# princeton-vl/DROID-SLAM

Measured on NVIDIA B200. Metric: BA-update iters/sec (512 edges, 344x64x48), higher is better.
Workload: dtype f32 (BA solve in f64), f16 corr volumes

## Files before the change

droid_slam_b200/csrc/ba.cu:

```cuda
#include "common.cuh"
#include "tcgen05.cuh"
#include <math.h>
#include <algorithm>

namespace dba {

constexpr int kBuildThreads = 256;
constexpr int kEdgeBatch = 16;

struct Layout {
  size_t off_hdr, off_frame2k, off_kx, off_rowptr, off_edgeidx, off_big, off_sys, off_L, off_dx, off_Eij, off_C, off_w, off_Ei, total;
  int P, n;
};

__host__ inline size_t align_up(size_t x, size_t a) { return (x + a - 1) / a * a; }

__host__ inline Layout make_layout(int N, int E, int ht, int wd, int t0, int t1) {
  Layout L;
  const size_t HW = (size_t)ht * wd;
  L.P = t1 - t0 > 0 ? t1 - t0 : 0;
  L.n = 6 * L.P;
  size_t o = 0;
  L.off_hdr = o;      o = align_up(o + 64 * sizeof(int), 256);
  L.off_frame2k = o;  o = align_up(o + (size_t)(N + 1) * sizeof(int), 256);
  L.off_kx = o;       o = align_up(o + (size_t)(N + 1) * sizeof(int), 256);
  L.off_rowptr = o;   o = align_up(o + (size_t)(N + 2) * sizeof(int), 256);
  L.off_edgeidx = o;  o = align_up(o + (size_t)(E + 1) * sizeof(int), 256);
  L.off_big = o;      o = align_up(o + (size_t)(N + 1) * sizeof(int), 256);
  L.off_sys = o;      o = align_up(o + ((size_t)L.n * L.n + L.n) * sizeof(double), 256);
  L.off_L = o;        o = align_up(o + chol_workspace_bytes(L.n), 256);
  L.off_dx = o;       o = align_up(o + (size_t)(L.n + 6) * sizeof(float), 256);
  L.off_Eij = o;      o = align_up(o + (size_t)E * 6 * HW * sizeof(float), 256);
  const size_t Mmax = (size_t)N;
  L.off_C = o;        o = align_up(o + Mmax * HW * sizeof(float), 256);
  L.off_w = o;        o = align_up(o + Mmax * HW * sizeof(float), 256);
  L.off_Ei = o;       o = align_up(o + Mmax * 6 * HW * sizeof(float), 256);
  L.total = o;
  return L;
}

enum { HDR_STATUS = 0, HDR_M = 1, HDR_CHOL_FAIL = 2, HDR_NBIG = 3 };
enum { ST_BAD_INDEX = 1, ST_ETA_ROWS = 2, ST_CHOL_FAIL = 4, ST_DEGREE = 8 };

__global__ void __launch_bounds__(1024) ba_prepare_kernel(const int64_t* __restrict__ ii, const int64_t* __restrict__ jj, int E, int N,
                                                          int t0, int t1, int eta_rows, int* __restrict__ hdr,
                                                          int* __restrict__ frame2k, int* __restrict__ kx, int* __restrict__ rowptr, int* __restrict__ big) {
  __shared__ int s_scan[1024];
  __shared__ int s_carry;
  const int tid = threadIdx.x;
  if (tid == 0) { hdr[HDR_STATUS] = 0; hdr[HDR_CHOL_FAIL] = 0; }
  for (int f = tid; f < N; f += blockDim.x) { frame2k[f] = (f >= t0 && f < t1) ? 1 : 0; rowptr[f] = 0; }
  if (tid == 0) { rowptr[N] = 0; rowptr[N + 1] = 0; }
  __syncthreads();
  for (int e = tid; e < E; e += blockDim.x) {
    const long long i = ii[e], j = jj[e];
    if (i < 0 || i >= N || j < 0 || j >= N) { atomicOr(&hdr[HDR_STATUS], ST_BAD_INDEX); continue; }
    frame2k[i] = 1;
  }
  __syncthreads();
  if (tid == 0) s_carry = 0;
  __syncthreads();
  for (int base = 0; base < N; base += blockDim.x) {
    const int f = base + tid;
    const int flag = (f < N) ? frame2k[f] : 0;
    s_scan[tid] = flag;
    __syncthreads();
    for (int off = 1; off < (int)blockDim.x; off <<= 1) {
      int v = (tid >= off) ? s_scan[tid - off] : 0;
      __syncthreads();
      s_scan[tid] += v;
      __syncthreads();
    }
    const int incl = s_scan[tid];
    const int idx = s_carry + incl - flag;
    if (f < N) {
      frame2k[f] = flag ? idx : -1;
      if (flag) kx[idx] = f;
    }
    __syncthreads();
    if (tid == blockDim.x - 1) s_carry += incl;
    __syncthreads();
  }
  const int M = s_carry;
  if (tid == 0) {
    hdr[HDR_M] = M;
    if (eta_rows != M && eta_rows != 1) atomicOr(&hdr[HDR_STATUS], ST_ETA_ROWS);
  }
  for (int e = tid; e < E; e += blockDim.x) {
    const long long i = ii[e], j = jj[e];
    if (i < 0 || i >= N || j < 0 || j >= N) continue;
    atomicAdd(&rowptr[frame2k[i] + 1], 1);
  }
  __syncthreads();
  if (tid == 0) s_carry = 0;
  __syncthreads();
  for (int base = 0; base <= M; base += blockDim.x) {
    const int m = base + tid;
    const int cnt = (m <= M) ? rowptr[m] : 0;
    s_scan[tid] = cnt;
    __syncthreads();
    for (int off = 1; off < (int)blockDim.x; off <<= 1) {
      int v = (tid >= off) ? s_scan[tid - off] : 0;
      __syncthreads();
      s_scan[tid] += v;
      __syncthreads();
    }
    if (m <= M) rowptr[m] = s_carry + s_scan[tid];
    __syncthreads();
    if (tid == blockDim.x - 1) s_carry += s_scan[tid];
    __syncthreads();
  }
  if (tid == 0) s_carry = 0;
  __syncthreads();
  for (int base = 0; base < M; base += blockDim.x) {
    const int m = base + tid;
    const int flag = (m < M && rowptr[m + 1] - rowptr[m] + 1 > 21) ? 1 : 0;
    s_scan[tid] = flag;
    __syncthreads();
    for (int off = 1; off < (int)blockDim.x; off <<= 1) {
      int v = (tid >= off) ? s_scan[tid - off] : 0;
      __syncthreads();
      s_scan[tid] += v;
      __syncthreads();
    }
    if (flag) big[s_carry + s_scan[tid] - 1] = m;
    __syncthreads();
    if (tid == blockDim.x - 1) s_carry += s_scan[tid];
    __syncthreads();
  }
  if (tid == 0) hdr[HDR_NBIG] = s_carry;
}

__global__ void __launch_bounds__(256) ba_fill_csr_kernel(const int64_t* __restrict__ ii, const int64_t* __restrict__ jj, int E, int N,
                                                          const int* __restrict__ frame2k, const int* __restrict__ rowptr,
                                                          int* __restrict__ edgeidx) {
  const int e = (blockIdx.x * blockDim.x + threadIdx.x) >> 5;
  const int lane = threadIdx.x & 31;
  if (e >= E) return;
  const long long i = ii[e], j = jj[e];
  if (i < 0 || i >= N || j < 0 || j >= N) return;
  int rank = 0;
  for (int f = lane; f < e; f += 32) {
    const long long i2 = ii[f], j2 = jj[f];
    rank += (i2 == i && j2 >= 0 && j2 < N) ? 1 : 0;
  }
// ... 22 lines not shown
  int e, jx, stereo;
};

__device__ __forceinline__ void adj_se3(const float* t, const float* q, const float* X, float* Y) {
  float qinv[4] = {-q[0], -q[1], -q[2], q[3]};
  act_so3(qinv, X, Y);
  act_so3(qinv, X + 3, Y + 3);
  float u[3], v[3];
  u[0] = t[2] * X[1] - t[1] * X[2];
  u[1] = t[0] * X[2] - t[2] * X[0];
  u[2] = t[1] * X[0] - t[0] * X[1];
  act_so3(qinv, u, v);
  Y[3] += v[0]; Y[4] += v[1]; Y[5] += v[2];
}

template <int kPPT>
__global__ void __launch_bounds__(kBuildThreads, 2) ba_build_kernel(
    const float* __restrict__ poses, const float* __restrict__ disps, const float* __restrict__ intr,
    const float* __restrict__ disps_sens, const float* __restrict__ targets, const float* __restrict__ weights,
    const float* __restrict__ eta, int eta_rows, int eta_by_frame, const int64_t* __restrict__ jj,
    const int* __restrict__ hdr, const int* __restrict__ kx, const int* __restrict__ rowptr, const int* __restrict__ edgeidx,
    int HW, int wd, int t0, int P, int motion_only,
    double* __restrict__ Hsys, double* __restrict__ bsys, float* __restrict__ Eij, float* __restrict__ Cout, float* __restrict__ wout,
    float* __restrict__ Eiout) {
  const int m = blockIdx.y;
  if (m >= hdr[HDR_M]) return;
  const int ix = kx[m];
  const int e_begin = rowptr[m], e_end = rowptr[m + 1];
  const int tid = threadIdx.x, lane = tid & 31, warp = tid >> 5;
  constexpr int NW = kBuildThreads / 32;

  __shared__ EdgeSm s_edge[kEdgeBatch];
  __shared__ float s_part[NW][kEdgeBatch][27];
  __shared__ double s_sum[kEdgeBatch][27];

  const float fx = __ldg(intr), fy = __ldg(intr + 1), cx = __ldg(intr + 2), cy = __ldg(intr + 3);
  const int n = 6 * P;

  int pix[kPPT];
  float Xi0[kPPT], Xi1[kPPT], dsp[kPPT];
  float Cacc[kPPT], wacc[kPPT], Eiacc[kPPT][6];
#pragma unroll
  for (int s = 0; s < kPPT; s++) {
    const int p = blockIdx.x * (kPPT * kBuildThreads) + s * kBuildThreads + tid;
    pix[s] = p;
    const bool ok = p < HW;
    const int i = ok ? p / wd : 0, j = ok ? p - i * wd : 0;
    Xi0[s] = ((float)j - cx) / fx;
    Xi1[s] = ((float)i - cy) / fy;
    dsp[s] = ok ? __ldg(disps + (size_t)ix * HW + p) : 1.f;
    Cacc[s] = 0.f; wacc[s] = 0.f;
#pragma unroll
    for (int c = 0; c < 6; c++) Eiacc[s][c] = 0.f;
  }

  for (int eb = e_begin; eb < e_end; eb += kEdgeBatch) {
    const int nb = min(kEdgeBatch, e_end - eb);
    __syncthreads();
    if (tid < nb) {
// ... 163 lines not shown
#pragma unroll
    for (int s = 0; s < kPPT; s++) {
      const int p = pix[s];
      if (p < HW) {
        const float dsn = __ldg(disps_sens + (size_t)ix * HW + p);
        const float mk = (dsn > 0.f) ? 1.f : 0.f;
        const float C = Cacc[s] + mk * alpha + (1 - mk) * __ldg(eta + (size_t)erow * HW + p);
        const float w = wacc[s] - mk * alpha * (dsp[s] - dsn);
        Cout[(size_t)m * HW + p] = C;
        wout[(size_t)m * HW + p] = w;
#pragma unroll
        for (int c = 0; c < 6; c++) Eiout[((size_t)m * 6 + c) * HW + p] = Eiacc[s][c];
      }
    }
  }
}

__device__ __forceinline__ float safe_rcp(float c) { return c > 0.f ? 1.0f / c : 0.f; }

constexpr int kSchurMaxRows = 255;

template <int kThreads>
__device__ __forceinline__ void build_row_list(const int64_t* __restrict__ jj, int* __restrict__ hdr, const int* __restrict__ edgeidx,
                                               int e_begin, int deg, int ix, int m, int HW, int t0, int P, const float* __restrict__ Eij,
                                               const float* __restrict__ Eiin, int* s_pose, const float** s_ptr, int* s_nrows, int* s_wcount) {
  const int tid = threadIdx.x, lane = tid & 31, warp = tid >> 5;
  const bool self = (ix >= t0 && ix < t0 + P);
  int pj = -1, e = -1;
  if (tid < deg && tid < kSchurMaxRows - 1) { e = edgeidx[e_begin + tid]; pj = (int)jj[e] - t0; }
  const bool keep = (pj >= 0 && pj < P);
  const unsigned bal = __ballot_sync(0xffffffffu, keep);
  if (lane == 0) s_wcount[warp] = __popc(bal);
  __syncthreads();
  int base = self ? 1 : 0;
  for (int w = 0; w < warp; w++) base += s_wcount[w];
// ... 280 lines not shown
    if (o < 36) {
      const int a = o / 6, c = o - a * 6;
      const int gr = pa_ * 6 + a, gc = pb_ * 6 + c;
      if (same_row) {
        if (gr >= gc) atomicAdd(&Hsys[(size_t)gr * n + gc], v);
      } else {
        if (gr >= gc) atomicAdd(&Hsys[(size_t)gr * n + gc], v);
        if (gc >= gr) atomicAdd(&Hsys[(size_t)gc * n + gr], v);
      }
    } else {
      atomicAdd(&bsys[pa_ * 6 + (o - 36)], v);
    }
  }
}

constexpr int kTcRowsMax = 21;
constexpr int kPairTileRows = 10;
constexpr int kPairRowsMax = 100;
constexpr int kPairGridZ = 45;
constexpr int kTcThreads = 288;
constexpr int kTcProducers = 256;
constexpr int kTcRawStages = 4;
constexpr int kTcRawBytes = 128 * 128;
constexpr int kTcOpBytes = 128 * 128;
constexpr int kTcOpStages = 4;
constexpr int kTcAccSlots = 3;
constexpr int kTcCxStride = 129;
constexpr int kTcSmem = kTcRawStages * kTcRawBytes + kTcOpStages * 2 * kTcOpBytes + 1024  + 256 ;
static_assert(128 * kTcCxStride * 4 <= kTcOpStages * 2 * kTcOpBytes, "G staging matrix must fit the operand ring");

__device__ __forceinline__ void cp_async16_zfill(uint32_t dst, const void* src, uint32_t src_bytes) {
  asm volatile("cp.async.cg.shared.global [%0], [%1], 16, %2;" ::"r"(dst), "l"(src), "r"(src_bytes) : "memory");
}
__device__ __forceinline__ float lds_f32(uint32_t addr) {
  float v;
  asm volatile("ld.shared.f32 %0, [%1];" : "=f"(v) : "r"(addr) : "memory");
  return v;
}
__device__ __forceinline__ void sts_f32(uint32_t addr, float v) { asm volatile("st.shared.f32 [%0], %1;" ::"r"(addr), "f"(v) : "memory"); }

template <bool PAIR>
__global__ void __launch_bounds__(kTcThreads, 1) ba_schur_tc_kernel(
    const int64_t* __restrict__ jj, int* __restrict__ hdr, const int* __restrict__ kx, const int* __restrict__ rowptr,
    const int* __restrict__ edgeidx, int HW, int t0, int P, int px_per_cta,
    const float* __restrict__ Eij, const float* __restrict__ Cin, const float* __restrict__ win, const float* __restrict__ Eiin,
    double* __restrict__ Hsys, double* __restrict__ bsys, const int* __restrict__ big) {
  if (PAIR && (int)blockIdx.y >= hdr[HDR_NBIG]) return;
  const int m = PAIR ? big[blockIdx.y] : blockIdx.y;
  if (m >= hdr[HDR_M]) return;
  const int ix = kx[m];
  const int e_begin = rowptr[m];
  const int deg = rowptr[m + 1] - e_begin;
  const int tid = threadIdx.x, lane = tid & 31, warp = tid >> 5;
  const int n = 6 * P;

  __shared__ int s_pose[kSchurMaxRows + 1];
  __shared__ const float* s_ptr[kSchurMaxRows + 1];
  __shared__ int s_nrows;
  __shared__ int s_wcount[kTcThreads / 32];
  __shared__ int s_gidx[128];
  extern __shared__ uint8_t tc_smem_raw[];

  if (deg == 0) return;
  if (PAIR) {
    if (deg + 1 <= kTcRowsMax) return;
    const int tmax = (min(deg + 1, kPairRowsMax) + kPairTileRows - 1) / kPairTileRows;
    if ((int)blockIdx.z >= tmax * (tmax - 1) / 2) return;
  }
  build_row_list<kTcThreads>(jj, hdr, edgeidx, e_begin, deg, ix, m, HW, t0, P, Eij, Eiin, s_pose, s_ptr, &s_nrows, s_wcount);
  const int nrows = s_nrows;
  if (!PAIR && (nrows == 0 || nrows > kTcRowsMax)) return;
  if (PAIR && (nrows <= kTcRowsMax || nrows > kPairRowsMax)) return;
  int ta = 0, tb = 0;
  bool emit_a = true, emit_b = true;
  if (PAIR) {
    const int T = (nrows + kPairTileRows - 1) / kPairTileRows;
    const int pr = blockIdx.z;
    if (pr >= T * (T - 1) / 2) return;
    tb = (int)((sqrtf(8.f * (float)pr + 1.f) + 1.f) * 0.5f);
    while (tb * (tb - 1) / 2 > pr) tb--;
    while ((tb + 1) * tb / 2 <= pr) tb++;
    ta = pr - tb * (tb - 1) / 2;
    emit_a = (tb == ta + 1);
    emit_b = (tb == T - 1 && ta == T - 2);
  }
  const int px_begin = blockIdx.x * px_per_cta;
  const int px_end = min(HW, px_begin + px_per_cta);
  if (px_begin >= px_end) return;
  const int R6a = PAIR ? 6 * min(kPairTileRows, nrows - kPairTileRows * ta) : 6 * nrows;
  const int R6b = PAIR ? 6 * min(kPairTileRows, nrows - kPairTileRows * tb) : 6 * nrows;
  const int R6 = R6a;
  const bool packed = !PAIR && (R6 + 2 <= 64);
  const bool two_halves = PAIR || packed;
  const int nhalf = packed ? 2 : 1;
  const int cpx = 32 * nhalf;
  const int nchunks = (px_end - px_begin + cpx - 1) / cpx;
  const int N = two_halves ? 128 : ((R6 + 1 + 15) & ~15);

  uint8_t* smem = reinterpret_cast<uint8_t*>((reinterpret_cast<uintptr_t>(tc_smem_raw) + 1023) & ~(uintptr_t)1023);
  const uint32_t op_base = smem_u32(smem);
  const uint32_t raw_base = op_base + kTcOpStages * 2 * kTcOpBytes;
  uint64_t* bars = reinterpret_cast<uint64_t*>(smem + kTcOpStages * 2 * kTcOpBytes + kTcRawStages * kTcRawBytes);
  uint64_t* full = bars;
  uint64_t* empty = bars + kTcOpStages;
  uint64_t* acc_full = bars + 2 * kTcOpStages;
  uint64_t* acc_empty = acc_full + kTcAccSlots;
  uint64_t* done = acc_empty + kTcAccSlots;
  uint32_t* tmem_base_smem = reinterpret_cast<uint32_t*>(done + 2);

  if (tid < 128) {
    if (PAIR) {
      const int hfx = tid >> 6, ln = tid & 63, R6x = hfx ? R6b : R6a, row0 = kPairTileRows * (hfx ? tb : ta);
      s_gidx[tid] = (ln < R6x) ? s_pose[row0 + ln / 6] * 6 + (ln % 6) : (ln == R6x ? -1 : -2);
    } else s_gidx[tid] = (tid < R6) ? s_pose[tid / 6] * 6 + (tid % 6) : (tid == R6 ? -1 : -2);
  }
  if (tid == 0) {
    for (int s = 0; s < kTcOpStages; s++) { mbar_init(full + s, kTcProducers / 32); mbar_init(empty + s, 1); }
    for (int s = 0; s < kTcAccSlots; s++) { mbar_init(acc_full + s, 1); mbar_init(acc_empty + s, kTcProducers / 32); }
    mbar_init(done, 1);
    asm volatile("fence.mbarrier_init.release.cluster;" ::: "memory");
  }
  if (warp == 8) {
    asm volatile("tcgen05.alloc.cta_group::1.sync.aligned.shared::cta.b32 [%0], 512;" ::"r"(smem_u32(tmem_base_smem)) : "memory");
    asm volatile("tcgen05.relinquish_alloc_permit.cta_group::1.sync.aligned;" ::: "memory");
  } else {
    uint4* z = reinterpret_cast<uint4*>(smem);
    for (int k = tid; k < kTcOpStages * 2 * kTcOpBytes / 16; k += kTcProducers) z[k] = make_uint4(0u, 0u, 0u, 0u);
  }
  asm volatile("tcgen05.fence::before_thread_sync;" ::: "memory");
  __syncthreads();
  asm volatile("tcgen05.fence::after_thread_sync;" ::: "memory");
  const uint32_t tmem_base = *tmem_base_smem;

  if (warp == 8) {
    if (lane == 0) {
      const uint32_t idesc = umma_idesc_tf32(128, N);
      const uint32_t d_g = tmem_base + 3 * 128;
      for (int c = 0; c < nchunks; c++) {
        const int os = c % kTcOpStages, slot = c % kTcAccSlots;
        mbar_wait(full + os, (c / kTcOpStages) & 1);
        if (c >= kTcAccSlots) mbar_wait(acc_empty + slot, ((c / kTcAccSlots) - 1) & 1);
        asm volatile("tcgen05.fence::after_thread_sync;" ::: "memory");
        const uint32_t hi0 = op_base + (uint32_t)os * 2 * kTcOpBytes, lo0 = hi0 + kTcOpBytes;
        const uint32_t d = tmem_base + (uint32_t)(slot * 128);
#pragma unroll
        for (int k = 0; k < 4; k++) {
          const uint64_t dh = umma_desc_k_sw128(hi0 + k * 32, 1024), dl = umma_desc_k_sw128(lo0 + k * 32, 1024);
          umma_tf32(d, dh, dh, idesc, k > 0 ? 1u : 0u);
          umma_tf32(d_g, dh, dl, idesc, (c > 0 || k > 0) ? 1u : 0u);
        }
        umma_commit(empty + os);
        umma_commit(acc_full + slot);
      }
      umma_commit(done);
    }
    __syncwarp();
  } else {
    const float* src[4];
    uint32_t dst[4];
    int pxo[4];
#pragma unroll
    for (int i = 0; i < 4; i++) {
      const int li = 4 * i + (lane >> 3), piece = lane & 7;
      const int hf = two_halves ? (li >> 3) : 0, line = warp + 8 * (two_halves ? (li & 7) : li);
      const int R6x = PAIR ? (hf ? R6b : R6a) : R6, row0 = PAIR ? kPairTileRows * (hf ? tb : ta) : 0;
      src[i] = Cin; pxo[i] = 1 << 30;
      dst[i] = raw_base + warp * 2048 + li * 128 + piece * 16;
      if (line <= R6x) {
        const float* base = (line < R6x) ? s_ptr[row0 + line / 6] + (size_t)(line % 6) * HW : win + (size_t)m * HW;
// ... 143 lines not shown
              if (gr > gc) atomicAdd(&Hsys[(size_t)gr * n + gc], v);
              else if (gr < gc) atomicAdd(&Hsys[(size_t)gc * n + gr], v);
              else atomicAdd(&Hsys[(size_t)gr * n + gr], 2.0 * v);
            } else if (gc >= 0) {
              if (gr >= gc) atomicAdd(&Hsys[(size_t)gr * n + gc], v);
            } else {
              atomicAdd(&bsys[gr], v);
            }
          }
        }
      }
    }
  }
  asm volatile("tcgen05.fence::before_thread_sync;" ::: "memory");
  __syncthreads();
  if (warp == 8) asm volatile("tcgen05.dealloc.cta_group::1.sync.aligned.b32 %0, 512;" ::"r"(tmem_base) : "memory");
}

__device__ __forceinline__ void exp_so3(const float* phi, float* q) {
  const float theta_sq = phi[0] * phi[0] + phi[1] * phi[1] + phi[2] * phi[2];
  const float theta_p4 = theta_sq * theta_sq;
  const float theta = sqrtf(theta_sq);
  float imag, real;
  if ((double)theta_sq < 1e-8) {
    imag = (float)(0.5 - (1.0 / 48.0) * (double)theta_sq + (1.0 / 3840.0) * (double)theta_p4);
    real = (float)(1.0 - (1.0 / 8.0) * (double)theta_sq + (1.0 / 384.0) * (double)theta_p4);
  } else {
    imag = (float)((double)sinf((float)(0.5 * (double)theta)) / (double)theta);
    real = cosf((float)(0.5 * (double)theta));
  }
// ... 107 lines not shown
  DBA_CHECK_ARG(a->p2p_world <= 8 && (a->p2p_world <= 1 || (a->p2p_rank >= 0 && a->p2p_rank < a->p2p_world)), "bad p2p rank/world");
  DBA_CHECK_ARG(a->workspace != nullptr, "null workspace");
  DBA_CHECK_ARG(a->n_frames <= 65535, "more than 65535 frames");
  L = make_layout(a->n_frames, a->n_edges, a->ht, a->wd, a->t0, a->t1);
  if (a->workspace_bytes < L.total) { dba::set_error("workspace too small: %zu < %zu", a->workspace_bytes, L.total); return DBA_ERR_WORKSPACE; }
  return DBA_OK;
}

#define WS(T, off) reinterpret_cast<T*>(reinterpret_cast<char*>(a->workspace) + (off))

static double* system_ptr(const dba_ba_args* a, const Layout& L) {
  if (a->p2p_world > 1) return reinterpret_cast<double*>(a->p2p_system[a->p2p_rank]) + (size_t)(a->p2p_epoch & 1ull) * ((size_t)L.n * L.n + L.n);
  return reinterpret_cast<double*>(reinterpret_cast<char*>(a->workspace) + L.off_sys);
}

extern "C" int dba_ba_prepare(const dba_ba_args* a) {
  Layout L; int rc = check_ba_args(a, L); if (rc) return rc;
  cudaStream_t st = (cudaStream_t)a->stream;
  ba_prepare_kernel<<<1, 1024, 0, st>>>(a->ii, a->jj, a->n_edges, a->n_frames, a->t0, a->t1, (a->motion_only || a->eta_by_frame) ? 1 : a->eta_rows,
                                        WS(int, L.off_hdr), WS(int, L.off_frame2k), WS(int, L.off_kx), WS(int, L.off_rowptr), WS(int, L.off_big));
  DBA_CHECK_LAUNCH("ba_prepare");
  if (a->n_edges > 0) {
    ba_fill_csr_kernel<<<(a->n_edges + 7) / 8, 256, 0, st>>>(a->ii, a->jj, a->n_edges, a->n_frames, WS(int, L.off_frame2k),
                                                                  WS(int, L.off_rowptr), WS(int, L.off_edgeidx));
    DBA_CHECK_LAUNCH("ba_fill_csr");
  }
  return DBA_OK;
}

extern "C" int dba_ba_build(const dba_ba_args* a) {
  Layout L; int rc = check_ba_args(a, L); if (rc) return rc;
  cudaStream_t st = (cudaStream_t)a->stream;
  const int HW = a->ht * a->wd;
  double* Hsys = system_ptr(a, L);
  double* bsys = Hsys + (size_t)L.n * L.n;
  DBA_CHECK_CUDA(cudaMemsetAsync(Hsys, 0, ((size_t)L.n * L.n + L.n) * sizeof(double), st), "ba_build memset");
  DBA_CHECK_CUDA(cudaMemsetAsync(WS(int, L.off_hdr) + HDR_CHOL_FAIL, 0, sizeof(int), st), "ba_build memset");
  if (L.P == 0) return DBA_OK;
  const int eff_frames = std::max(1, std::min(a->n_frames, a->own_hi - a->own_lo));
  const int ppt = (eff_frames * ((HW + 4 * kBuildThreads - 1) / (4 * kBuildThreads)) >= 148) ? 4
                : (eff_frames * ((HW + 2 * kBuildThreads - 1) / (2 * kBuildThreads)) >= 148) ? 2 : 1;
#define LAUNCH_BUILD(PPT)                                                                                                               \
  ba_build_kernel<PPT><<<dim3((HW + PPT * kBuildThreads - 1) / (PPT * kBuildThreads), a->n_frames), kBuildThreads, 0, st>>>(             \
      a->poses, a->disps, a->intrinsics, a->disps_sens, a->targets, a->weights, a->eta, a->eta_rows, a->eta_by_frame, a->jj, WS(int, L.off_hdr),  \
      WS(int, L.off_kx), WS(int, L.off_rowptr), WS(int, L.off_edgeidx), HW, a->wd, a->t0, L.P, a->motion_only, Hsys, bsys,               \
      WS(float, L.off_Eij), WS(float, L.off_C), WS(float, L.off_w), WS(float, L.off_Ei))
  if (ppt == 4) LAUNCH_BUILD(4); else if (ppt == 2) LAUNCH_BUILD(2); else LAUNCH_BUILD(1);
#undef LAUNCH_BUILD
  DBA_CHECK_LAUNCH("ba_build");
  if (!a->motion_only) {
    const size_t smem2 = (size_t)2 * kSgK * kSgStride * sizeof(float);
    const int tiles1 = (HW + kSgK - 1) / kSgK;
    const int chunks1 = std::max(1, std::min(tiles1, (5 * 148 / 2 + eff_frames - 1) / eff_frames));
    const int px_per_cta1 = ((tiles1 + chunks1 - 1) / chunks1) * kSgK;
    const int gx1 = (HW + px_per_cta1 - 1) / px_per_cta1;
    const int px_per_cta2 = ((HW + 2) / 3 + kSgK - 1) / kSgK * kSgK;
    const int gx2 = (HW + px_per_cta2 - 1) / px_per_cta2;
    const int zsplit2 = std::max(1, std::min(32, (6 * 148 + eff_frames * gx2 - 1) / (eff_frames * gx2)));
    if ((rc = kernel_setup((const void*)ba_schur_gemm_kernel, (int)smem2))) return rc;
    if ((rc = kernel_setup((const void*)ba_schur_small_kernel, (int)smem2))) return rc;
    if ((rc = kernel_setup((const void*)ba_schur_tc_kernel<false>, (int)kTcSmem))) return rc;
    if ((rc = kernel_setup((const void*)ba_schur_tc_kernel<true>, (int)kTcSmem))) return rc;
    const bool use_tc = HW % 4 == 0;
    if (use_tc) {
      const int tiles64 = (HW + 63) / 64;
      const int chunks_tc = std::max(1, std::min(tiles64, (148 + eff_frames / 2) / eff_frames));
      const int px_per_cta_tc = ((tiles64 + chunks_tc - 1) / chunks_tc) * 64;
      const int gx_tc = (HW + px_per_cta_tc - 1) / px_per_cta_tc;
      ba_schur_tc_kernel<false><<<dim3(gx_tc, a->n_frames, 1), kTcThreads, kTcSmem, st>>>(a->jj, WS(int, L.off_hdr), WS(int, L.off_kx), WS(int, L.off_rowptr),
                                                           WS(int, L.off_edgeidx), HW, a->t0, L.P, px_per_cta_tc, WS(float, L.off_Eij),
                                                           WS(float, L.off_C), WS(float, L.off_w), WS(float, L.off_Ei), Hsys, bsys, WS(int, L.off_big));
      const int max_big = std::min(a->n_frames, a->n_edges / kTcRowsMax);
      if (max_big > 0)
        ba_schur_tc_kernel<true><<<dim3(1, max_big, kPairGridZ), kTcThreads, kTcSmem, st>>>(a->jj, WS(int, L.off_hdr), WS(int, L.off_kx), WS(int, L.off_rowptr),
                                                           WS(int, L.off_edgeidx), HW, a->t0, L.P, ((HW + 31) / 32) * 32, WS(float, L.off_Eij),
                                                           WS(float, L.off_C), WS(float, L.off_w), WS(float, L.off_Ei), Hsys, bsys, WS(int, L.off_big));
    } else {
      ba_schur_small_kernel<<<dim3(gx1, a->n_frames, 1), kSgThreads, smem2, st>>>(a->jj, WS(int, L.off_hdr), WS(int, L.off_kx), WS(int, L.off_rowptr),
                                                           WS(int, L.off_edgeidx), HW, a->t0, L.P, px_per_cta1, WS(float, L.off_Eij),
                                                           WS(float, L.off_C), WS(float, L.off_w), WS(float, L.off_Ei), Hsys, bsys);
    }
    DBA_CHECK_LAUNCH("ba_schur<single>");
    ba_schur_gemm_kernel<<<dim3(gx2, a->n_frames, zsplit2), kSgThreads, smem2, st>>>(a->jj, WS(int, L.off_hdr), WS(int, L.off_kx), WS(int, L.off_rowptr),
                                                                         WS(int, L.off_edgeidx), HW, a->t0, L.P, px_per_cta2, use_tc ? kPairRowsMax : kSgRows, WS(float, L.off_Eij),
                                                                         WS(float, L.off_C), WS(float, L.off_w), WS(float, L.off_Ei), Hsys, bsys);
    DBA_CHECK_LAUNCH("ba_schur<multi>");
  }
  return DBA_OK;
}

extern "C" int dba_ba_solve(const dba_ba_args* a) {
// ... 78 lines not shown
```

Before: 873.1.

## Use persistent work-queue kernels for BA build and tensor-core Schur stages

```diff
diff --git a/droid_slam_b200/csrc/ba.cu b/droid_slam_b200/csrc/ba.cu
--- a/droid_slam_b200/csrc/ba.cu
+++ b/droid_slam_b200/csrc/ba.cu
@@ -2,16 +2,31 @@
 #include "tcgen05.cuh"
 #include <math.h>
 #include <algorithm>
+#include <climits>
 
 namespace dba {
 
 constexpr int kBuildThreads = 256;
 constexpr int kEdgeBatch = 16;
+constexpr int kPPT = 4;
+constexpr int kBuildCtasPerSm = 2;
+constexpr int kSchurMaxRows = 255;
+constexpr int kTcPackedRowsMax = 10;
+constexpr int kTcRowsMax = 21;
+constexpr int kPairTileRows = 10;
+constexpr int kPairRowsMax = 100;
+constexpr int kTcItemOverhead = 4;
 
 struct Layout {
-  size_t off_hdr, off_frame2k, off_kx, off_rowptr, off_edgeidx, off_big, off_sys, off_L, off_dx, off_Eij, off_C, off_w, off_Ei, total;
+  size_t off_hdr, off_frame2k, off_kx, off_rowptr, off_edgeidx, off_rows, off_work, off_bwork, off_sys, off_L, off_dx, off_Eij, off_C, off_w, off_Ei, total;
   int P, n;
 };
+
+constexpr int kTcRangesMax = 64;
+constexpr int kPairItemsMax = 45;
+__host__ inline size_t tc_work_capacity(int N, int E) {
+  return (size_t)N * kTcRangesMax + (size_t)std::min(N, E / 21) * kPairItemsMax;
+}
 
 __host__ inline size_t align_up(size_t x, size_t a) { return (x + a - 1) / a * a; }
 
@@ -26,7 +41,9 @@
   L.off_kx = o;       o = align_up(o + (size_t)(N + 1) * sizeof(int), 256);
   L.off_rowptr = o;   o = align_up(o + (size_t)(N + 2) * sizeof(int), 256);
   L.off_edgeidx = o;  o = align_up(o + (size_t)(E + 1) * sizeof(int), 256);
-  L.off_big = o;      o = align_up(o + (size_t)(N + 1) * sizeof(int), 256);
+  L.off_rows = o;     o = align_up(o + (size_t)(N + 1) * sizeof(int), 256);
+  L.off_work = o;     o = align_up(o + tc_work_capacity(N, E) * sizeof(int4), 256);
+  L.off_bwork = o;    o = align_up(o + (size_t)N * ((HW + 255) / 256) * sizeof(int4), 256);
   L.off_sys = o;      o = align_up(o + ((size_t)L.n * L.n + L.n) * sizeof(double), 256);
   L.off_L = o;        o = align_up(o + chol_workspace_bytes(L.n), 256);
   L.off_dx = o;       o = align_up(o + (size_t)(L.n + 6) * sizeof(float), 256);
@@ -39,96 +56,168 @@
   return L;
 }
 
-enum { HDR_STATUS = 0, HDR_M = 1, HDR_CHOL_FAIL = 2, HDR_NBIG = 3 };
+enum { HDR_STATUS = 0, HDR_M = 1, HDR_CHOL_FAIL = 2, HDR_NEXT = 3, HDR_BNEXT = 4, HDR_NWORK = 5, HDR_NBWORK = 6 };
 enum { ST_BAD_INDEX = 1, ST_ETA_ROWS = 2, ST_CHOL_FAIL = 4, ST_DEGREE = 8 };
 
+__device__ __forceinline__ int block_scan_excl(int v, int* s_warp, int* total) {
+  const int tid = threadIdx.x, lane = tid & 31, warp = tid >> 5;
+  int x = v;
+#pragma unroll
+  for (int o = 1; o < 32; o <<= 1) { const int y = __shfl_up_sync(0xffffffffu, x, o); if (lane >= o) x += y; }
+  if (lane == 31) s_warp[warp] = x;
+  __syncthreads();
+  if (warp == 0) {
+    int w = s_warp[lane];
+#pragma unroll
+    for (int o = 1; o < 32; o <<= 1) { const int y = __shfl_up_sync(0xffffffffu, w, o); if (lane >= o) w += y; }
+    s_warp[lane] = w - s_warp[lane];
+    if (lane == 31) s_warp[32] = w;
+  }
+  __syncthreads();
+  const int r = s_warp[warp] + x - v;
+  *total = s_warp[32];
+  __syncthreads();
+  return r;
+}
+
+__device__ __forceinline__ int tc_chunks(int R, int deg, int HW) {
+  if (deg == 0 || deg > kSchurMaxRows - 1 || R == 0 || R > kTcRowsMax) return 0;
+  return R <= kTcPackedRowsMax ? (HW + 63) / 64 : (HW + 31) / 32;
+}
+__device__ __forceinline__ int tc_pairs(int R, int deg) {
+  if (deg > kSchurMaxRows - 1 || R <= kTcRowsMax || R > kPairRowsMax) return 0;
+  const int T = (R + kPairTileRows - 1) / kPairTileRows;
+  return T * (T - 1) / 2;
+}
+
+__device__ __forceinline__ int build_ppt(int deg, int cmax4) {
+  return (deg * 4 <= cmax4) ? 4 : (deg * 2 <= cmax4) ? 2 : 1;
+}
+
 __global__ void __launch_bounds__(1024) ba_prepare_kernel(const int64_t* __restrict__ ii, const int64_t* __restrict__ jj, int E, int N,
-                                                          int t0, int t1, int eta_rows, int* __restrict__ hdr,
-                                                          int* __restrict__ frame2k, int* __restrict__ kx, int* __restrict__ rowptr, int* __restrict__ big) {
-  __shared__ int s_scan[1024];
-  __shared__ int s_carry;
+                                                          int t0, int t1, int eta_rows, int HW, int tc_grid, int build_slots,
+                                                          int* __restrict__ hdr, int* __restrict__ frame2k, int* __restrict__ kx,
+                                                          int* __restrict__ rowptr, int* __restrict__ rows, int4* __restrict__ work,
+                                                          int4* __restrict__ bwork) {
+  __shared__ int s_warp[33];
+  __shared__ int s_cnt[2];
+  __shared__ int s_cpi;
   const int tid = threadIdx.x;
-  if (tid == 0) { hdr[HDR_STATUS] = 0; hdr[HDR_CHOL_FAIL] = 0; }
-  for (int f = tid; f < N; f += blockDim.x) { frame2k[f] = (f >= t0 && f < t1) ? 1 : 0; rowptr[f] = 0; }
+  const int nthr = blockDim.x;
+  if (tid == 0) { hdr[HDR_STATUS] = 0; hdr[HDR_CHOL_FAIL] = 0; s_cnt[0] = 0; s_cnt[1] = 0; }
+  for (int f = tid; f < N; f += nthr) { frame2k[f] = (f >= t0 && f < t1) ? 1 : 0; rowptr[f] = 0; }
   if (tid == 0) { rowptr[N] = 0; rowptr[N + 1] = 0; }
   __syncthreads();
-  for (int e = tid; e < E; e += blockDim.x) {
+  for (int e = tid; e < E; e += nthr) {
     const long long i = ii[e], j = jj[e];
     if (i < 0 || i >= N || j < 0 || j >= N) { atomicOr(&hdr[HDR_STATUS], ST_BAD_INDEX); continue; }
     frame2k[i] = 1;
   }
   __syncthreads();
-  if (tid == 0) s_carry = 0;
-  __syncthreads();
-  for (int base = 0; base < N; base += blockDim.x) {
+  int carry = 0, tot;
+  for (int base = 0; base < N; base += nthr) {
     const int f = base + tid;
     const int flag = (f < N) ? frame2k[f] : 0;
-    s_scan[tid] = flag;
-    __syncthreads();
-    for (int off = 1; off < (int)blockDim.x; off <<= 1) {
-      int v = (tid >= off) ? s_scan[tid - off] : 0;
-      __syncthreads();
-      s_scan[tid] += v;
-      __syncthreads();
-    }
-    const int incl = s_scan[tid];
-    const int idx = s_carry + incl - flag;
+    const int idx = carry + block_scan_excl(flag, s_warp, &tot);
     if (f < N) {
       frame2k[f] = flag ? idx : -1;
       if (flag) kx[idx] = f;
     }
-    __syncthreads();
-    if (tid == blockDim.x - 1) s_carry += incl;
-    __syncthreads();
-  }
-  const int M = s_carry;
+    carry += tot;
+  }
+  const int M = carry;
   if (tid == 0) {
     hdr[HDR_M] = M;
     if (eta_rows != M && eta_rows != 1) atomicOr(&hdr[HDR_STATUS], ST_ETA_ROWS);
   }
-  for (int e = tid; e < E; e += blockDim.x) {
+  __syncthreads();
+  for (int m = tid; m < M; m += nthr) rows[m] = (kx[m] >= t0 && kx[m] < t1) ? 1 : 0;
+  __syncthreads();
+  for (int e = tid; e < E; e += nthr) {
     const long long i = ii[e], j = jj[e];
     if (i < 0 || i >= N || j < 0 || j >= N) continue;
     atomicAdd(&rowptr[frame2k[i] + 1], 1);
-  }
-  __syncthreads();
-  if (tid == 0) s_carry = 0;
-  __syncthreads();
-  for (int base = 0; base <= M; base += blockDim.x) {
+    if (j >= t0 && j < t1) atomicAdd(&rows[frame2k[i]], 1);
+  }
+  __syncthreads();
+  carry = 0;
+  for (int base = 0; base <= M; base += nthr) {
     const int m = base + tid;
     const int cnt = (m <= M) ? rowptr[m] : 0;
-    s_scan[tid] = cnt;
-    __syncthreads();
-    for (int off = 1; off < (int)blockDim.x; off <<= 1) {
-      int v = (tid >= off) ? s_scan[tid - off] : 0;
-      __syncthreads();
-      s_scan[tid] += v;
-      __syncthreads();
-    }
-    if (m <= M) rowptr[m] = s_carry + s_scan[tid];
-    __syncthreads();
-    if (tid == blockDim.x - 1) s_carry += s_scan[tid];
-    __syncthreads();
-  }
-  if (tid == 0) s_carry = 0;
-  __syncthreads();
-  for (int base = 0; base < M; base += blockDim.x) {
-    const int m = base + tid;
-    const int flag = (m < M && rowptr[m + 1] - rowptr[m] + 1 > 21) ? 1 : 0;
-    s_scan[tid] = flag;
-    __syncthreads();
-    for (int off = 1; off < (int)blockDim.x; off <<= 1) {
-      int v = (tid >= off) ? s_scan[tid - off] : 0;
-      __syncthreads();
-      s_scan[tid] += v;
-      __syncthreads();
-    }
-    if (flag) big[s_carry + s_scan[tid] - 1] = m;
-    __syncthreads();
-    if (tid == blockDim.x - 1) s_carry += s_scan[tid];
-    __syncthreads();
-  }
-  if (tid == 0) hdr[HDR_NBIG] = s_carry;
+    const int incl = carry + block_scan_excl(cnt, s_warp, &tot) + cnt;
+    if (m <= M) rowptr[m] = incl;
+    carry += tot;
+  }
+  __syncthreads();
+
+  {
+    int w = 0;
+    for (int m = tid; m < M; m += nthr) w += max(1, rowptr[m + 1] - rowptr[m]);
+    const int chunks4 = (HW + 1023) / 1024;
+    int wsum = 0;
+    block_scan_excl(w, s_warp, &wsum);
+    const int cmax4 = max(16, (int)(4LL * wsum * chunks4 / max(1, build_slots)));
+    carry = 0;
+    for (int base = 0; base < M; base += nthr) {
+      const int m = base + tid;
+      int cnt = 0, px = 0;
+      if (m < M) {
+        px = 256 * build_ppt(rowptr[m + 1] - rowptr[m], cmax4);
+        cnt = (HW + px - 1) / px;
+      }
+      const int first = carry + block_scan_excl(cnt, s_warp, &tot);
+      for (int r = 0; r < cnt; r++) bwork[first + r] = make_int4(m, r * px, min(HW, (r + 1) * px), 0);
+      carry += tot;
+    }
+    if (tid == 0) hdr[HDR_NBWORK] = carry;
+  }
+
+  if (tc_grid <= 0) { if (tid == 0) hdr[HDR_NWORK] = 0; return; }
+  for (int m = tid; m < M; m += nthr) {
+    const int R = rows[m], deg = rowptr[m + 1] - rowptr[m];
+    if (tc_chunks(R, deg, HW)) atomicAdd(&s_cnt[R <= kTcPackedRowsMax ? 0 : 1], 1);
+  }
+  __syncthreads();
+  if (tid < 32) {
+    const int cp = (HW + 63) / 64, cu = (HW + 31) / 32;
+    const int cpi_min = (cu + kTcRangesMax - 1) / kTcRangesMax;
+    long long best_cost = LLONG_MAX; int best = 0;
+    for (int c = tid + 1; c <= 64; c += 32) {
+      const long long items = (long long)s_cnt[0] * ((cp + c - 1) / c) + (long long)s_cnt[1] * ((cu + c - 1) / c);
+      const long long cost = c < cpi_min ? LLONG_MAX : (items + tc_grid - 1) / tc_grid * (c + kTcItemOverhead);
+      if (cost < best_cost || (cost == best_cost && c > best)) { best_cost = cost; best = c; }
+    }
+#pragma unroll
+    for (int o = 16; o > 0; o >>= 1) {
+      const long long oc = __shfl_xor_sync(0xffffffffu, best_cost, o);
+      const int ob = __shfl_xor_sync(0xffffffffu, best, o);
+      if (oc < best_cost || (oc == best_cost && ob > best)) { best_cost = oc; best = ob; }
+    }
+    if (tid == 0) s_cpi = max(best, cpi_min);
+  }
+  __syncthreads();
+  const int cpi = s_cpi;
+  carry = 0;
+  for (int pass = 0; pass < 2; pass++) {
+    for (int base = 0; base < M; base += nthr) {
+      const int m = base + tid;
+      int cnt = 0, R = 0, deg = 0;
+      if (m < M) {
+        R = rows[m]; deg = rowptr[m + 1] - rowptr[m];
+        cnt = pass == 0 ? tc_pairs(R, deg) : (tc_chunks(R, deg, HW) + cpi - 1) / cpi;
+      }
+      const int first = carry + block_scan_excl(cnt, s_warp, &tot);
+      if (pass == 0) {
+        for (int z = 0; z < cnt; z++) work[first + z] = make_int4(m, 0, HW, z);
+      } else if (cnt > 0) {
+        const int c = tc_chunks(R, deg, HW), cpx = R <= kTcPackedRowsMax ? 64 : 32;
+        for (int r = 0; r < cnt; r++)
+          work[first + r] = make_int4(m, (int)((long long)r * c / cnt) * cpx, min(HW, (int)((long long)(r + 1) * c / cnt) * cpx), -1);
+      }
+      carry += tot;
+    }
+  }
+  if (tid == 0) hdr[HDR_NWORK] = carry;
 }
 
 __global__ void __launch_bounds__(256) ba_fill_csr_kernel(const int64_t* __restrict__ ii, const int64_t* __restrict__ jj, int E, int N,
@@ -181,35 +270,43 @@
   Y[3] += v[0]; Y[4] += v[1]; Y[5] += v[2];
 }
 
-template <int kPPT>
-__global__ void __launch_bounds__(kBuildThreads, 2) ba_build_kernel(
+__global__ void __launch_bounds__(kBuildThreads, kBuildCtasPerSm) ba_build_kernel(
     const float* __restrict__ poses, const float* __restrict__ disps, const float* __restrict__ intr,
     const float* __restrict__ disps_sens, const float* __restrict__ targets, const float* __restrict__ weights,
     const float* __restrict__ eta, int eta_rows, int eta_by_frame, const int64_t* __restrict__ jj,
-    const int* __restrict__ hdr, const int* __restrict__ kx, const int* __restrict__ rowptr, const int* __restrict__ edgeidx,
+    int* __restrict__ hdr, const int* __restrict__ kx, const int* __restrict__ rowptr, const int* __restrict__ edgeidx,
     int HW, int wd, int t0, int P, int motion_only,
     double* __restrict__ Hsys, double* __restrict__ bsys, float* __restrict__ Eij, float* __restrict__ Cout, float* __restrict__ wout,
-    float* __restrict__ Eiout) {
-  const int m = blockIdx.y;
-  if (m >= hdr[HDR_M]) return;
-  const int ix = kx[m];
-  const int e_begin = rowptr[m], e_end = rowptr[m + 1];
+    float* __restrict__ Eiout, const int4* __restrict__ bwork) {
   const int tid = threadIdx.x, lane = tid & 31, warp = tid >> 5;
   constexpr int NW = kBuildThreads / 32;
 
   __shared__ EdgeSm s_edge[kEdgeBatch];
   __shared__ float s_part[NW][kEdgeBatch][27];
   __shared__ double s_sum[kEdgeBatch][27];
+  __shared__ int s_item;
 
   const float fx = __ldg(intr), fy = __ldg(intr + 1), cx = __ldg(intr + 2), cy = __ldg(intr + 3);
   const int n = 6 * P;
+  const int nwork = hdr[HDR_NBWORK];
+  for (;;) {
+  __syncthreads();
+  if (tid == 0) s_item = atomicAdd(&hdr[HDR_BNEXT], 1);
+  __syncthreads();
+  const int item = s_item;
+  if (item >= nwork) break;
+  const int4 wk = bwork[item];
+  const int m = wk.x, px_end = wk.z;
+  const int ix = kx[m];
+  const int e_begin = rowptr[m], e_end = rowptr[m + 1];
 
   int pix[kPPT];
   float Xi0[kPPT], Xi1[kPPT], dsp[kPPT];
   float Cacc[kPPT], wacc[kPPT], Eiacc[kPPT][6];
 #pragma unroll
   for (int s = 0; s < kPPT; s++) {
-    const int p = blockIdx.x * (kPPT * kBuildThreads) + s * kBuildThreads + tid;
+    const int p0 = wk.y + s * kBuildThreads + tid;
+    const int p = p0 < px_end ? p0 : HW;
     pix[s] = p;
     const bool ok = p < HW;
     const int i = ok ? p / wd : 0, j = ok ? p - i * wd : 0;
@@ -403,11 +500,11 @@
       }
     }
   }
+  }
 }
 
 __device__ __forceinline__ float safe_rcp(float c) { return c > 0.f ? 1.0f / c : 0.f; }
 
-constexpr int kSchurMaxRows = 255;
 
 template <int kThreads>
 __device__ __forceinline__ void build_row_list(const int64_t* __restrict__ jj, int* __restrict__ hdr, const int* __restrict__ edgeidx,
@@ -718,10 +815,6 @@
   }
 }
 
-constexpr int kTcRowsMax = 21;
-constexpr int kPairTileRows = 10;
-constexpr int kPairRowsMax = 100;
-constexpr int kPairGridZ = 45;
 constexpr int kTcThreads = 288;
 constexpr int kTcProducers = 256;
 constexpr int kTcRawStages = 4;
@@ -743,44 +836,39 @@
 }
 __device__ __forceinline__ void sts_f32(uint32_t addr, float v) { asm volatile("st.shared.f32 [%0], %1;" ::"r"(addr), "f"(v) : "memory"); }
 
+struct TcShared {
+  int pose[kSchurMaxRows + 1];
+  const float* ptr[kSchurMaxRows + 1];
+  int nrows;
+  int wcount[kTcThreads / 32];
+  int gidx[128];
+};
+
 template <bool PAIR>
-__global__ void __launch_bounds__(kTcThreads, 1) ba_schur_tc_kernel(
+__device__ __forceinline__ bool schur_tc_item(
     const int64_t* __restrict__ jj, int* __restrict__ hdr, const int* __restrict__ kx, const int* __restrict__ rowptr,
-    const int* __restrict__ edgeidx, int HW, int t0, int P, int px_per_cta,
+    const int* __restrict__ edgeidx, int HW, int t0, int P, int m, int px_begin, int px_end, int pr,
     const float* __restrict__ Eij, const float* __restrict__ Cin, const float* __restrict__ win, const float* __restrict__ Eiin,
-    double* __restrict__ Hsys, double* __restrict__ bsys, const int* __restrict__ big) {
-  if (PAIR && (int)blockIdx.y >= hdr[HDR_NBIG]) return;
-  const int m = PAIR ? big[blockIdx.y] : blockIdx.y;
-  if (m >= hdr[HDR_M]) return;
+    double* __restrict__ Hsys, double* __restrict__ bsys, TcShared& sh, uint8_t* smem, uint32_t tmem_base) {
   const int ix = kx[m];
   const int e_begin = rowptr[m];
   const int deg = rowptr[m + 1] - e_begin;
   const int tid = threadIdx.x, lane = tid & 31, warp = tid >> 5;
   const int n = 6 * P;
-
-  __shared__ int s_pose[kSchurMaxRows + 1];
-  __shared__ const float* s_ptr[kSchurMaxRows + 1];
-  __shared__ int s_nrows;
-  __shared__ int s_wcount[kTcThreads / 32];
-  __shared__ int s_gidx[128];
-  extern __shared__ uint8_t tc_smem_raw[];
-
-  if (deg == 0) return;
-  if (PAIR) {
-    if (deg + 1 <= kTcRowsMax) return;
-    const int tmax = (min(deg + 1, kPairRowsMax) + kPairTileRows - 1) / kPairTileRows;
-    if ((int)blockIdx.z >= tmax * (tmax - 1) / 2) return;
-  }
-  build_row_list<kTcThreads>(jj, hdr, edgeidx, e_begin, deg, ix, m, HW, t0, P, Eij, Eiin, s_pose, s_ptr, &s_nrows, s_wcount);
-  const int nrows = s_nrows;
-  if (!PAIR && (nrows == 0 || nrows > kTcRowsMax)) return;
-  if (PAIR && (nrows <= kTcRowsMax || nrows > kPairRowsMax)) return;
+  int* s_pose = sh.pose;
+  const float** s_ptr = sh.ptr;
+  int* s_gidx = sh.gidx;
+
+  if (deg == 0) return false;
+  build_row_list<kTcThreads>(jj, hdr, edgeidx, e_begin, deg, ix, m, HW, t0, P, Eij, Eiin, s_pose, s_ptr, &sh.nrows, sh.wcount);
+  const int nrows = sh.nrows;
+  if (!PAIR && (nrows == 0 || nrows > kTcRowsMax)) return false;
+  if (PAIR && (nrows <= kTcRowsMax || nrows > kPairRowsMax)) return false;
   int ta = 0, tb = 0;
   bool emit_a = true, emit_b = true;
   if (PAIR) {
     const int T = (nrows + kPairTileRows - 1) / kPairTileRows;
-    const int pr = blockIdx.z;
-    if (pr >= T * (T - 1) / 2) return;
+    if (pr >= T * (T - 1) / 2) return false;
     tb = (int)((sqrtf(8.f * (float)pr + 1.f) + 1.f) * 0.5f);
     while (tb * (tb - 1) / 2 > pr) tb--;
     while ((tb + 1) * tb / 2 <= pr) tb++;
@@ -788,9 +876,7 @@
     emit_a = (tb == ta + 1);
     emit_b = (tb == T - 1 && ta == T - 2);
   }
-  const int px_begin = blockIdx.x * px_per_cta;
-  const int px_end = min(HW, px_begin + px_per_cta);
-  if (px_begin >= px_end) return;
+  if (px_begin >= px_end) return false;
   const int R6a = PAIR ? 6 * min(kPairTileRows, nrows - kPairTileRows * ta) : 6 * nrows;
   const int R6b = PAIR ? 6 * min(kPairTileRows, nrows - kPairTileRows * tb) : 6 * nrows;
   const int R6 = R6a;
@@ -801,7 +887,6 @@
   const int nchunks = (px_end - px_begin + cpx - 1) / cpx;
   const int N = two_halves ? 128 : ((R6 + 1 + 15) & ~15);
 
-  uint8_t* smem = reinterpret_cast<uint8_t*>((reinterpret_cast<uintptr_t>(tc_smem_raw) + 1023) & ~(uintptr_t)1023);
   const uint32_t op_base = smem_u32(smem);
   const uint32_t raw_base = op_base + kTcOpStages * 2 * kTcOpBytes;
   uint64_t* bars = reinterpret_cast<uint64_t*>(smem + kTcOpStages * 2 * kTcOpBytes + kTcRawStages * kTcRawBytes);
@@ -810,7 +895,6 @@
   uint64_t* acc_full = bars + 2 * kTcOpStages;
   uint64_t* acc_empty = acc_full + kTcAccSlots;
   uint64_t* done = acc_empty + kTcAccSlots;
-  uint32_t* tmem_base_smem = reinterpret_cast<uint32_t*>(done + 2);
 
   if (tid < 128) {
     if (PAIR) {
@@ -818,23 +902,7 @@
       s_gidx[tid] = (ln < R6x) ? s_pose[row0 + ln / 6] * 6 + (ln % 6) : (ln == R6x ? -1 : -2);
     } else s_gidx[tid] = (tid < R6) ? s_pose[tid / 6] * 6 + (tid % 6) : (tid == R6 ? -1 : -2);
   }
-  if (tid == 0) {
-    for (int s = 0; s < kTcOpStages; s++) { mbar_init(full + s, kTcProducers / 32); mbar_init(empty + s, 1); }
-    for (int s = 0; s < kTcAccSlots; s++) { mbar_init(acc_full + s, 1); mbar_init(acc_empty + s, kTcProducers / 32); }
-    mbar_init(done, 1);
-    asm volatile("fence.mbarrier_init.release.cluster;" ::: "memory");
-  }
-  if (warp == 8) {
-    asm volatile("tcgen05.alloc.cta_group::1.sync.aligned.shared::cta.b32 [%0], 512;" ::"r"(smem_u32(tmem_base_smem)) : "memory");
-    asm volatile("tcgen05.relinquish_alloc_permit.cta_group::1.sync.aligned;" ::: "memory");
-  } else {
-    uint4* z = reinterpret_cast<uint4*>(smem);
-    for (int k = tid; k < kTcOpStages * 2 * kTcOpBytes / 16; k += kTcProducers) z[k] = make_uint4(0u, 0u, 0u, 0u);
-  }
-  asm volatile("tcgen05.fence::before_thread_sync;" ::: "memory");
-  __syncthreads();
-  asm volatile("tcgen05.fence::after_thread_sync;" ::: "memory");
-  const uint32_t tmem_base = *tmem_base_smem;
+  __syncthreads();
 
   if (warp == 8) {
     if (lane == 0) {
@@ -857,6 +925,7 @@
         umma_commit(acc_full + slot);
       }
       umma_commit(done);
+      for (int c = max(0, nchunks - kTcOpStages); c < nchunks; c++) mbar_wait(empty + c % kTcOpStages, (c / kTcOpStages) & 1);
     }
     __syncwarp();
   } else {
@@ -1030,6 +1099,69 @@
   }
   asm volatile("tcgen05.fence::before_thread_sync;" ::: "memory");
   __syncthreads();
+  asm volatile("tcgen05.fence::after_thread_sync;" ::: "memory");
+  return true;
+}
+
+__device__ __forceinline__ void tc_init_barriers(uint64_t* bars, bool reinit) {
+  uint64_t* full = bars;
+  uint64_t* empty = bars + kTcOpStages;
+  uint64_t* acc_full = bars + 2 * kTcOpStages;
+  uint64_t* acc_empty = acc_full + kTcAccSlots;
+  uint64_t* done = acc_empty + kTcAccSlots;
+  if (reinit)
+    for (int s = 0; s < 2 * kTcOpStages + 2 * kTcAccSlots + 1; s++) asm volatile("mbarrier.inval.shared::cta.b64 [%0];" ::"r"(smem_u32(bars + s)) : "memory");
+  for (int s = 0; s < kTcOpStages; s++) { mbar_init(full + s, kTcProducers / 32); mbar_init(empty + s, 1); }
+  for (int s = 0; s < kTcAccSlots; s++) { mbar_init(acc_full + s, 1); mbar_init(acc_empty + s, kTcProducers / 32); }
+  mbar_init(done, 1);
+  asm volatile("fence.mbarrier_init.release.cluster;" ::: "memory");
+}
+
+__global__ void __launch_bounds__(kTcThreads, 1) ba_schur_tc_kernel(
+    const int64_t* __restrict__ jj, int* __restrict__ hdr, const int* __restrict__ kx, const int* __restrict__ rowptr,
+    const int* __restrict__ edgeidx, int HW, int t0, int P, const int4* __restrict__ work,
+    const float* __restrict__ Eij, const float* __restrict__ Cin, const float* __restrict__ win, const float* __restrict__ Eiin,
+    double* __restrict__ Hsys, double* __restrict__ bsys) {
+  __shared__ TcShared sh;
+  __shared__ int s_item;
+  extern __shared__ uint8_t tc_smem_raw[];
+  const int tid = threadIdx.x, warp = tid >> 5;
+  const int nwork = hdr[HDR_NWORK];
+  if (tid == 0) s_item = atomicAdd(&hdr[HDR_NEXT], 1);
+  __syncthreads();
+  int item = s_item;
+  if (item >= nwork) return;
+
+  uint8_t* smem = reinterpret_cast<uint8_t*>((reinterpret_cast<uintptr_t>(tc_smem_raw) + 1023) & ~(uintptr_t)1023);
+  uint64_t* bars = reinterpret_cast<uint64_t*>(smem + kTcOpStages * 2 * kTcOpBytes + kTcRawStages * kTcRawBytes);
+  uint32_t* tmem_base_smem = reinterpret_cast<uint32_t*>(bars + 2 * kTcOpStages + 2 * kTcAccSlots + 2);
+  if (tid == 0) tc_init_barriers(bars, false);
+  if (warp == 8) {
+    asm volatile("tcgen05.alloc.cta_group::1.sync.aligned.shared::cta.b32 [%0], 512;" ::"r"(smem_u32(tmem_base_smem)) : "memory");
+    asm volatile("tcgen05.relinquish_alloc_permit.cta_group::1.sync.aligned;" ::: "memory");
+  } else {
+    uint4* z = reinterpret_cast<uint4*>(smem);
+    for (int k = tid; k < kTcOpStages * 2 * kTcOpBytes / 16; k += kTcProducers) z[k] = make_uint4(0u, 0u, 0u, 0u);
+  }
+  asm volatile("tcgen05.fence::before_thread_sync;" ::: "memory");
+  __syncthreads();
+  asm volatile("tcgen05.fence::after_thread_sync;" ::: "memory");
+  const uint32_t tmem_base = *tmem_base_smem;
+
+  while (item < nwork) {
+    const int4 w = work[item];
+    const bool used = w.w < 0 ? schur_tc_item<false>(jj, hdr, kx, rowptr, edgeidx, HW, t0, P, w.x, w.y, w.z, 0, Eij, Cin, win, Eiin, Hsys, bsys, sh, smem, tmem_base)
+                              : schur_tc_item<true>(jj, hdr, kx, rowptr, edgeidx, HW, t0, P, w.x, w.y, w.z, w.w, Eij, Cin, win, Eiin, Hsys, bsys, sh, smem, tmem_base);
+    __syncthreads();
+    if (tid == 0) {
+      if (used) tc_init_barriers(bars, true);
+      s_item = atomicAdd(&hdr[HDR_NEXT], 1);
+    }
+    __syncthreads();
+    item = s_item;
+  }
+  asm volatile("tcgen05.fence::before_thread_sync;" ::: "memory");
+  __syncthreads();
   if (warp == 8) asm volatile("tcgen05.dealloc.cta_group::1.sync.aligned.b32 %0, 512;" ::"r"(tmem_base) : "memory");
 }
 
@@ -1167,11 +1299,26 @@
   return reinterpret_cast<double*>(reinterpret_cast<char*>(a->workspace) + L.off_sys);
 }
 
+static int tc_schur_grid(const dba_ba_args* a, const Layout& L, int* grid) {
+  *grid = 0;
+  if (a->motion_only || L.P == 0 || (a->ht * a->wd) % 4 != 0) return DBA_OK;
+  DeviceInfo di;
+  int rc = device_info(&di);
+  if (rc) return rc;
+  *grid = di.num_sms;
+  return DBA_OK;
+}
+
 extern "C" int dba_ba_prepare(const dba_ba_args* a) {
   Layout L; int rc = check_ba_args(a, L); if (rc) return rc;
   cudaStream_t st = (cudaStream_t)a->stream;
+  int tc_grid = 0;
+  if ((rc = tc_schur_grid(a, L, &tc_grid))) return rc;
+  DeviceInfo di;
+  if ((rc = device_info(&di))) return rc;
   ba_prepare_kernel<<<1, 1024, 0, st>>>(a->ii, a->jj, a->n_edges, a->n_frames, a->t0, a->t1, (a->motion_only || a->eta_by_frame) ? 1 : a->eta_rows,
-                                        WS(int, L.off_hdr), WS(int, L.off_frame2k), WS(int, L.off_kx), WS(int, L.off_rowptr), WS(int, L.off_big));
+                                        a->ht * a->wd, tc_grid, kBuildCtasPerSm * di.num_sms, WS(int, L.off_hdr), WS(int, L.off_frame2k),
+                                        WS(int, L.off_kx), WS(int, L.off_rowptr), WS(int, L.off_rows), WS(int4, L.off_work), WS(int4, L.off_bwork));
   DBA_CHECK_LAUNCH("ba_prepare");
   if (a->n_edges > 0) {
     ba_fill_csr_kernel<<<(a->n_edges + 7) / 8, 256, 0, st>>>(a->ii, a->jj, a->n_edges, a->n_frames, WS(int, L.off_frame2k),
@@ -1188,18 +1335,16 @@
   double* Hsys = system_ptr(a, L);
   double* bsys = Hsys + (size_t)L.n * L.n;
   DBA_CHECK_CUDA(cudaMemsetAsync(Hsys, 0, ((size_t)L.n * L.n + L.n) * sizeof(double), st), "ba_build memset");
-  DBA_CHECK_CUDA(cudaMemsetAsync(WS(int, L.off_hdr) + HDR_CHOL_FAIL, 0, sizeof(int), st), "ba_build memset");
+  static_assert(HDR_NEXT == HDR_CHOL_FAIL + 1 && HDR_BNEXT == HDR_CHOL_FAIL + 2, "one memset resets the three words");
+  DBA_CHECK_CUDA(cudaMemsetAsync(WS(int, L.off_hdr) + HDR_CHOL_FAIL, 0, 3 * sizeof(int), st), "ba_build memset");
   if (L.P == 0) return DBA_OK;
+  DeviceInfo di;
+  if ((rc = device_info(&di))) return rc;
+  ba_build_kernel<<<kBuildCtasPerSm * di.num_sms, kBuildThreads, 0, st>>>(
+      a->poses, a->disps, a->intrinsics, a->disps_sens, a->targets, a->weights, a->eta, a->eta_rows, a->eta_by_frame, a->jj, WS(int, L.off_hdr),
+      WS(int, L.off_kx), WS(int, L.off_rowptr), WS(int, L.off_edgeidx), HW, a->wd, a->t0, L.P, a->motion_only, Hsys, bsys,
+      WS(float, L.off_Eij), WS(float, L.off_C), WS(float, L.off_w), WS(float, L.off_Ei), WS(int4, L.off_bwork));
   const int eff_frames = std::max(1, std::min(a->n_frames, a->own_hi - a->own_lo));
-  const int ppt = (eff_frames * ((HW + 4 * kBuildThreads - 1) / (4 * kBuildThreads)) >= 148) ? 4
-                : (eff_frames * ((HW + 2 * kBuildThreads - 1) / (2 * kBuildThreads)) >= 148) ? 2 : 1;
-#define LAUNCH_BUILD(PPT)                                                                                                               \
-  ba_build_kernel<PPT><<<dim3((HW + PPT * kBuildThreads - 1) / (PPT * kBuildThreads), a->n_frames), kBuildThreads, 0, st>>>(             \
-      a->poses, a->disps, a->intrinsics, a->disps_sens, a->targets, a->weights, a->eta, a->eta_rows, a->eta_by_frame, a->jj, WS(int, L.off_hdr),  \
-      WS(int, L.off_kx), WS(int, L.off_rowptr), WS(int, L.off_edgeidx), HW, a->wd, a->t0, L.P, a->motion_only, Hsys, bsys,               \
-      WS(float, L.off_Eij), WS(float, L.off_C), WS(float, L.off_w), WS(float, L.off_Ei))
-  if (ppt == 4) LAUNCH_BUILD(4); else if (ppt == 2) LAUNCH_BUILD(2); else LAUNCH_BUILD(1);
-#undef LAUNCH_BUILD
   DBA_CHECK_LAUNCH("ba_build");
   if (!a->motion_only) {
     const size_t smem2 = (size_t)2 * kSgK * kSgStride * sizeof(float);
@@ -1212,22 +1357,14 @@
     const int zsplit2 = std::max(1, std::min(32, (6 * 148 + eff_frames * gx2 - 1) / (eff_frames * gx2)));
     if ((rc = kernel_setup((const void*)ba_schur_gemm_kernel, (int)smem2))) return rc;
     if ((rc = kernel_setup((const void*)ba_schur_small_kernel, (int)smem2))) return rc;
-    if ((rc = kernel_setup((const void*)ba_schur_tc_kernel<false>, (int)kTcSmem))) return rc;
-    if ((rc = kernel_setup((const void*)ba_schur_tc_kernel<true>, (int)kTcSmem))) return rc;
-    const bool use_tc = HW % 4 == 0;
+    if ((rc = kernel_setup((const void*)ba_schur_tc_kernel, (int)kTcSmem))) return rc;
+    int tc_grid = 0;
+    if ((rc = tc_schur_grid(a, L, &tc_grid))) return rc;
+    const bool use_tc = tc_grid > 0;
     if (use_tc) {
-      const int tiles64 = (HW + 63) / 64;
-      const int chunks_tc = std::max(1, std::min(tiles64, (148 + eff_frames / 2) / eff_frames));
-      const int px_per_cta_tc = ((tiles64 + chunks_tc - 1) / chunks_tc) * 64;
-      const int gx_tc = (HW + px_per_cta_tc - 1) / px_per_cta_tc;
-      ba_schur_tc_kernel<false><<<dim3(gx_tc, a->n_frames, 1), kTcThreads, kTcSmem, st>>>(a->jj, WS(int, L.off_hdr), WS(int, L.off_kx), WS(int, L.off_rowptr),
-                                                           WS(int, L.off_edgeidx), HW, a->t0, L.P, px_per_cta_tc, WS(float, L.off_Eij),
-                                                           WS(float, L.off_C), WS(float, L.off_w), WS(float, L.off_Ei), Hsys, bsys, WS(int, L.off_big));
-      const int max_big = std::min(a->n_frames, a->n_edges / kTcRowsMax);
-      if (max_big > 0)
-        ba_schur_tc_kernel<true><<<dim3(1, max_big, kPairGridZ), kTcThreads, kTcSmem, st>>>(a->jj, WS(int, L.off_hdr), WS(int, L.off_kx), WS(int, L.off_rowptr),
-                                                           WS(int, L.off_edgeidx), HW, a->t0, L.P, ((HW + 31) / 32) * 32, WS(float, L.off_Eij),
-                                                           WS(float, L.off_C), WS(float, L.off_w), WS(float, L.off_Ei), Hsys, bsys, WS(int, L.off_big));
+      ba_schur_tc_kernel<<<tc_grid, kTcThreads, kTcSmem, st>>>(a->jj, WS(int, L.off_hdr), WS(int, L.off_kx), WS(int, L.off_rowptr), WS(int, L.off_edgeidx),
+                                                               HW, a->t0, L.P, WS(int4, L.off_work), WS(float, L.off_Eij), WS(float, L.off_C),
+                                                               WS(float, L.off_w), WS(float, L.off_Ei), Hsys, bsys);
     } else {
       ba_schur_small_kernel<<<dim3(gx1, a->n_frames, 1), kSgThreads, smem2, st>>>(a->jj, WS(int, L.off_hdr), WS(int, L.off_kx), WS(int, L.off_rowptr),
                                                            WS(int, L.off_edgeidx), HW, a->t0, L.P, px_per_cta1, WS(float, L.off_Eij),
```

Result: no change. 880.7, median of 6 (+0.9%).
